# RoboticExplorationLab/TortoiseSat.jl

Hardware: AMD Instinct MI355X
Metric: AL-iLQR trajectory solves/sec (1000 knots) (higher is better)
Workload: dtype f64

## Files before the change

### tortoisesat.jl_amd/csrc/tsat_device.hpp

```cpp
#pragma once
#include <stdint.h>
#include "../../include/tortoise_hip.h"

#ifdef TSAT_EMU
#include <cmath>
namespace tsat_emu { int lane(); void sync(); void* lds(); double* xch(); }
#define TSAT_DEV inline
#define TSAT_PHASE inline
#define TSAT_FWD inline
#define TSAT_GLOBAL
#define TSAT_CONSTMEM
#define TSAT_LANE() (tsat_emu::lane())
#define TSAT_SYNC() (tsat_emu::sync())
#define TSAT_SYNC_LDS() (tsat_emu::sync())
#define TSAT_SCHED_FENCE() ((void)0)
#define TSAT_WAIT_LDS() ((void)0)
#define TSAT_NO_UNROLL
#define TSAT_ATOMIC_ADD(ptr, v) __atomic_fetch_add((ptr), (v), __ATOMIC_RELAXED)
#define TSAT_ATOMIC_LOAD(ptr) __atomic_load_n((ptr), __ATOMIC_RELAXED)
#define TSAT_UNIFORM_INT(x) (x)
#define TSAT_LANES_BELOW(n) (true)
#else
#define TSAT_DEV __device__ __forceinline__
#define TSAT_PHASE __device__ __noinline__
// ... 86 lines not shown
#elif defined(TSAT_JAC32)
  static constexpr int CHB = 64;
#elif defined(TSAT_DENSE)
  static constexpr int CHB = ES ? 29 : 25;
#else
  static constexpr int CHB = ES ? 64 : 55;
#endif
};
constexpr int KDW = 24, XUW = 10, LMW = 6, BSW = 9;
template <typename real> constexpr size_t pad16(size_t n) { return (n + (16 / sizeof(real)) - 1) / (16 / sizeof(real)) * (16 / sizeof(real)); }
template <typename real> constexpr size_t xu_stride(int NS) { return pad16<real>((size_t)NS * XUW); }
template <typename real> constexpr size_t kd_stride(int NS) { return (size_t)(NS - 1) * KDW; }
template <typename real> constexpr size_t lam_stride(int NS) { return pad16<real>((size_t)(NS - 1) * LMW); }
template <typename real> constexpr size_t u0_stride(int NS) { return (size_t)(NS - 1) * 3; }

template <typename real>
struct KArgs {
  int T, N, n_tab, max_ls;
  tsat_options opt;
  const real* P;
  const real* BT;
  const int* bidx;
  const int* nk;
  const real* U0;
  real* XU;
  real* KD;
  real* LAM;
  real* CAND;
  tsat_stats* stats;
  double* trace;
  int trace_rows;
  real* JW;
  int pk_few = 0;
  int ls_few = N_FEW, ls_hold = LS_HOLD;
  int suspend_at = 0;
  int* live = nullptr;
  int* susp_n = nullptr;
  int* susp_ids = nullptr;
  void* susp_state = nullptr;
};

constexpr int TSAT_JW_REALS_PER_4 = 16 * (4 * 84 + 4);

template <typename real>
struct TPtrs {
  TSAT_GLOBAL real* XU;
  TSAT_GLOBAL real* KD;
  TSAT_GLOBAL real* LAM;
  TSAT_GLOBAL real* CAND;
  const TSAT_GLOBAL real* bt;
  TSAT_GLOBAL real* XU0;
  int cur;
};
TSAT_DEV int cand_slab(int cur, int c) { return (c < cur) ? c : c + 1; }
template <typename real>
TSAT_DEV TSAT_GLOBAL real* slab_ptr(const TPtrs<real>& p, int N, int id) {
  return (id == 0) ? p.XU0 : p.CAND + (size_t)(id - 1) * (size_t)N * XUW;
}

constexpr int L_RED = 0;
constexpr int L_TR = L_RED + 64;
constexpr int TR_HJI = PSTRIDE, TR_HH = PSTRIDE + 9, TR_US = PSTRIDE + 10;
constexpr int L_NU = L_TR + 76;
constexpr int L_PC = L_NU + 8;
constexpr int L_ST = L_PC + 4;
constexpr int L_WT = L_ST + 72;
constexpr int L_HXX = L_WT + 90;
constexpr int L_HUX = L_HXX + 50;
constexpr int L_HUU = L_HUX + 24;
constexpr int L_KD = L_HUU + 10;
constexpr int L_ZERO = L_KD + 24;
constexpr int L_SINK = L_ZERO + 1;
constexpr int L_UNION = L_SINK + 1;
static_assert(L_UNION % 2 == 0, "phase buffers must stay 16-byte aligned");
constexpr int L_REC = L_UNION;
constexpr int GLDS = RPU * WAVE;
constexpr int BROW_UNITS = 4 / RPU;
constexpr int FB_KD = 0;
constexpr int FB_XU = FB_KD + ((CK * KDW + GLDS - 1) / GLDS) * GLDS;
constexpr int FB_BA = FB_XU + ((CK * XUW + GLDS - 1) / GLDS) * GLDS;
constexpr int FB_BB = FB_BA + ((CK * 3 * RPU + GLDS - 1) / GLDS) * GLDS;
constexpr int FB_SIZE = FB_BB + (BROW_UNITS == 2 ? ((CK * 3 * RPU + GLDS - 1) / GLDS) * GLDS : 0);
constexpr int CG = 2, KB = 4 * WAVE, KBS = KB + 2;
#if defined(TSAT_DENSE) || (defined(TSAT_F32) && TSAT_OCC >= 3)
constexpr int FWD_NBUF = 1;
#else
constexpr int FWD_NBUF = 2;
#endif
constexpr int L_FWD = L_UNION;
constexpr int L_FWD_END = L_FWD + (FWD_NBUF * FB_SIZE > CG * KBS ? FWD_NBUF * FB_SIZE : CG * KBS);
constexpr int L_BWD_RECV = (BwdCfg<0>::CHB * BwdCfg<0>::RECS > BwdCfg<1>::CHB * BwdCfg<1>::RECS
                               ? BwdCfg<0>::CHB * BwdCfg<0>::RECS : BwdCfg<1>::CHB * BwdCfg<1>::RECS);
constexpr int L_BWD_SOLVE = (L_BWD_RECV * (int)sizeof(jac_t) + (int)sizeof(cfg_real) - 1) / (int)sizeof(cfg_real);
#if !defined(TSAT_DENSE) && !defined(TSAT_F32)
constexpr int L_BWD_END = L_REC + (L_BWD_SOLVE > TV_CHB * TvRec::RECS ? L_BWD_SOLVE : TV_CHB * TvRec::RECS);
#else
constexpr int L_BWD_END = L_REC + L_BWD_SOLVE;
#endif
#if defined(TSAT_PACKED)
#ifndef TSAT_PK_LDS_BYTES
#define TSAT_PK_LDS_BYTES 20480
#endif
constexpr int LDS_REALS = (TSAT_PK_LDS_BYTES - ((sizeof(cfg_real) == 8) ? 0 : 64 * 8)) / (int)sizeof(cfg_real);
#else
constexpr int LDS_REALS = (L_FWD_END > L_BWD_END ? L_FWD_END : L_BWD_END);
#endif

constexpr int RED64_BYTES = (sizeof(cfg_real) == 8) ? 0 : 64 * 8;
constexpr int LDS_BYTES = LDS_REALS * (int)sizeof(cfg_real) + RED64_BYTES;
#ifndef TSAT_EMU
__shared__ __align__(16) unsigned char tsat_smem[LDS_BYTES];
#endif
template <typename real>
TSAT_DEV real* lds_base() {
  static_assert(sizeof(real) == sizeof(cfg_real), "the LDS carve-up is counted in the translation unit's storage type");
#ifdef TSAT_EMU
  return reinterpret_cast<real*>(tsat_emu::lds());
#else
  return reinterpret_cast<real*>(tsat_smem);
#endif
}
TSAT_DEV acc_t* red64() {
#ifdef TSAT_EMU
  unsigned char* b = reinterpret_cast<unsigned char*>(tsat_emu::lds());
#else
  unsigned char* b = tsat_smem;
#endif
  return reinterpret_cast<acc_t*>(b + (RED64_BYTES ? LDS_REALS * (int)sizeof(cfg_real) : L_RED * (int)sizeof(cfg_real)));
}

TSAT_DEV double* st64() {
#ifdef TSAT_EMU
  unsigned char* b = reinterpret_cast<unsigned char*>(tsat_emu::lds());
#else
  unsigned char* b = tsat_smem;
#endif
  return reinterpret_cast<double*>(b + L_ST * (int)sizeof(cfg_real));
}

template <typename real> TSAT_DEV real rsqrt_(real s);
#ifdef TSAT_EMU
template <> TSAT_DEV double rsqrt_<double>(double s) { return 1.0 / std::sqrt(s); }
template <> TSAT_DEV float rsqrt_<float>(float s) { return 1.0f / std::sqrt(s); }
TSAT_DEV double fabs_(double a) { return std::fabs(a); }
TSAT_DEV double fmax_(double a, double b) { return a > b ? a : b; }
TSAT_DEV double fmaxabs_(double a, double b) { const double c = std::fabs(b); return a > c ? a : c; }
TSAT_DEV double floor_(double a) { return std::floor(a); }
TSAT_DEV double fma_(double a, double b, double c) { return std::fma(a, b, c); }
TSAT_DEV double rcp_(double a) { return 1.0 / a; }
TSAT_DEV double sqrt_(double a) { return std::sqrt(a); }
TSAT_DEV double sin_(double a) { return std::sin(a); }
TSAT_DEV double cos_(double a) { return std::cos(a); }
TSAT_DEV double acos_(double a) { return std::acos(a); }
TSAT_DEV double asin_(double a) { return std::asin(a); }
TSAT_DEV double atan2_(double a, double b) { return std::atan2(a, b); }
TSAT_DEV double fmod_(double a, double b) { return std::fmod(a, b); }
TSAT_DEV double log_(double a) { return std::log(a); }
TSAT_DEV float fabs_(float a) { return std::fabs(a); }
TSAT_DEV float fmax_(float a, float b) { return a > b ? a : b; }
TSAT_DEV float fmaxabs_(float a, float b) { const float c = std::fabs(b); return a > c ? a : c; }
TSAT_DEV float rcp_(float a) { return 1.0f / a; }
TSAT_DEV float fma_(float a, float b, float c) { return std::fma(a, b, c); }
#else
template <> TSAT_DEV double rsqrt_<double>(double s) {
  const double y = __builtin_amdgcn_rsq(s);
  const double e = __builtin_fma(-(s * y), y, 1.0);
  const double p = __builtin_fma(0.375, e, 0.5) * e;
  return __builtin_fma(y, p, y);
}
template <> TSAT_DEV float rsqrt_<float>(float s) { return __builtin_amdgcn_rsqf(s); }
TSAT_DEV double fabs_(double a) { return __builtin_fabs(a); }
TSAT_DEV double fmax_(double a, double b) { double r; asm("v_max_f64 %0, %1, %2" : "=v"(r) : "v"(a), "v"(b)); return r; }
TSAT_DEV double fmaxabs_(double a, double b) { double r; asm("v_max_f64 %0, %1, |%2|" : "=v"(r) : "v"(a), "v"(b)); return r; }
TSAT_DEV double floor_(double a) { return __builtin_floor(a); }
TSAT_DEV double fma_(double a, double b, double c) { return __builtin_fma(a, b, c); }
TSAT_DEV double rcp_(double a) {
  const double y = __builtin_amdgcn_rcp(a);
  const double e = __builtin_fma(-a, y, 1.0);
  const double p = __builtin_fma(e, e, e);
  return __builtin_fma(y, p, y);
}
TSAT_DEV double sqrt_(double a) { return __builtin_sqrt(a); }
TSAT_DEV double sin_(double a) { return ::sin(a); }
TSAT_DEV double cos_(double a) { return ::cos(a); }
TSAT_DEV double acos_(double a) { return ::acos(a); }
TSAT_DEV double asin_(double a) { return ::asin(a); }
TSAT_DEV double atan2_(double a, double b) { return ::atan2(a, b); }
TSAT_DEV double fmod_(double a, double b) { return ::fmod(a, b); }
TSAT_DEV double log_(double a) { return ::log(a); }
TSAT_DEV float fabs_(float a) { return __builtin_fabsf(a); }
TSAT_DEV float fmax_(float a, float b) { float r; asm("v_max_f32 %0, %1, %2" : "=v"(r) : "v"(a), "v"(b)); return r; }
TSAT_DEV float fmaxabs_(float a, float b) { float r; asm("v_max_f32 %0, %1, |%2|" : "=v"(r) : "v"(a), "v"(b)); return r; }
TSAT_DEV float rcp_(float a) { return __builtin_amdgcn_rcpf(a); }
TSAT_DEV float fma_(float a, float b, float c) { return __builtin_fmaf(a, b, c); }
#endif
template <typename real> TSAT_DEV real dmm_(real a, real b, real c, real d) { return fma_(a, b, -(c * d)); }
template <typename real> TSAT_DEV real dot3_(real a0, real b0, real a1, real b1, real a2, real b2) { return fma_(a2, b2, fma_(a1, b1, a0 * b0)); }

#if defined(TSAT_PROFILE) && !defined(TSAT_EMU)
TSAT_DEV unsigned long long tick_() { return __builtin_amdgcn_s_memtime(); }
TSAT_DEV unsigned long long wall_() { return wall_clock64(); }
#else
TSAT_DEV unsigned long long tick_() { return 0ull; }
TSAT_DEV unsigned long long wall_() { return 0ull; }
#endif

template <typename real>
TSAT_DEV real sel7(const real a[7], int i) {
  real v = a[0];
  for (int m = 1; m < 7; ++m) v = (i == m) ? a[m] : v;
  return v;
}

template <typename real> TSAT_DEV real inf_() { return (real)__builtin_huge_val(); }

template <typename real>
TSAT_DEV void role_store(real* lds, int off, int sink, real v) {
#ifdef TSAT_EMU
  if (off == sink) return;
#else
  (void)sink;
#endif
  lds[off] = v;
}

template <typename real>
TSAT_DEV real wave_sum(real v, real* red) {
  const int lane = TSAT_LANE();
  for (int s = 1; s < WAVE; s <<= 1) {
    red[lane] = v;
    TSAT_SYNC_LDS();
    v = v + red[lane ^ s];
    TSAT_SYNC_LDS();
  }
  return v;
}
template <typename real>
TSAT_DEV real wave_max(real v, real* red) {
  const int lane = TSAT_LANE();
  for (int s = 1; s < WAVE; s <<= 1) {
    red[lane] = v;
    TSAT_SYNC_LDS();
    real o = red[lane ^ s];
    v = (o > v) ? o : v;
    TSAT_SYNC_LDS();
  }
  return v;
}
template <typename real>
TSAT_DEV real wave_bcast(real v, int src, real* red) {
  const int lane = TSAT_LANE();
  if (lane == src) red[0] = v;
  TSAT_SYNC_LDS();
  real r = red[0];
  TSAT_SYNC_LDS();
  return r;
}
template <typename real>
TSAT_DEV int wave_first(bool flag, real* red) {
  real v = flag ? (real)TSAT_LANE() : (real)WAVE;
  const int lane = TSAT_LANE();
  for (int s = 1; s < WAVE; s <<= 1) {
    red[lane] = v;
    TSAT_SYNC_LDS();
    real o = red[lane ^ s];
    v = (o < v) ? o : v;
    TSAT_SYNC_LDS();
  }
  return (int)v;
}

template <typename real>
struct Traj {
  real xf[7], Qd[7], Qfd[7], Rd[3], ulo[3], uhi[3];
  real J[9];
  real hJi[9];
  real h, hh, us;
  real usj;
  double tau0, dtau;
  int N, n_tab;
  const TSAT_GLOBAL real* bt;
};

template <typename real>
TSAT_DEV Traj<real> load_traj_at(const real* t, int N, int n_tab, const TSAT_GLOBAL real* bt) {
  Traj<real> tr;
  for (int i = 0; i < 7; ++i) { tr.xf[i] = t[P_XF + i]; tr.Qd[i] = t[P_QD + i]; tr.Qfd[i] = t[P_QFD + i]; }
  for (int i = 0; i < 3; ++i) { tr.Rd[i] = t[P_RD + i]; tr.ulo[i] = t[P_ULO + i]; tr.uhi[i] = t[P_UHI + i]; }
  for (int i = 0; i < 9; ++i) { tr.J[i] = t[P_J + i]; tr.hJi[i] = t[TR_HJI + i]; }
  tr.h = t[P_DT]; tr.hh = t[TR_HH]; tr.us = t[TR_US]; tr.usj = tr.us * tr.hJi[0];
  tr.tau0 = (double)t[P_TAU0] + (double)t[P_TAU0L]; tr.dtau = (double)t[P_DTAU] + (double)t[P_DTAUL];
  tr.N = N; tr.n_tab = n_tab; tr.bt = bt;
  return tr;
}
template <typename real>
TSAT_DEV Traj<real> load_traj(int N, int n_tab, const TSAT_GLOBAL real* bt) {
  return load_traj_at<real>(lds_base<real>() + L_TR, N, n_tab, bt);
// ... 440 lines not shown
  for (int i = 0; i < 7; ++i) x[i] = lds[L_TR + P_X0 + i];
  const TSAT_GLOBAL real* XUg = p.XU;
  const TSAT_GLOBAL real* KDg = p.KD;
  TSAT_GLOBAL real* Cg = slab_ptr<real>(p, N, cand_slab(p.cur, lane < n_cand ? lane : 0));
  int cur = 0;
  fwd_chunk_issue<real>(lds + L_FWD, KDg, XUg, tr, 0, (N - 1 < CK) ? N - 1 : CK, closed);
  TSAT_SYNC();
  for (int k0 = 0; k0 < N - 1; k0 += CK) {
    const int nk = (N - 1 - k0 < CK) ? (N - 1 - k0) : CK;
    const int kn = k0 + CK, nkn = (N - 1 - kn < CK) ? (N - 1 - kn) : CK;
    real* fb = lds + L_FWD + cur * FB_SIZE;
    real* fbn = lds + L_FWD + ((FWD_NBUF == 2) ? (1 - cur) : 0) * FB_SIZE;
    if (FWD_NBUF == 2 && nkn > 0) fwd_chunk_issue<real>(fbn, KDg, XUg, tr, kn, nkn, closed);
    auto knot = [&](const KnotIn<real>& kin, int kk) {
      const real* xu = kin.xu;
      real u[3] = {xu[7], xu[8], xu[9]};
      if (closed) {
        const real* kd = kin.kd;
        real dx[7];
        if (ES) {
          for (int i = 0; i < 3; ++i) dx[i] = x[i] - xu[i];
          const real s1 = xu[3], a1 = -xu[4], a2 = -xu[5], a3 = -xu[6];
          const real s2 = x[3], b1 = x[4], b2 = x[5], b3 = x[6];
          const real e0 = s1 * s2 - (a1 * b1 + a2 * b2 + a3 * b3);
          const real e1 = s1 * b1 + s2 * a1 + (a2 * b3 - a3 * b2);
          const real e2 = s1 * b2 + s2 * a2 + (a3 * b1 - a1 * b3);
          const real e3 = s1 * b3 + s2 * a3 + (a1 * b2 - a2 * b1);
          const real ir = rcp_((real)1 + e0);
          dx[3] = e1 * ir; dx[4] = e2 * ir; dx[5] = e3 * ir; dx[6] = 0;
        } else {
          for (int i = 0; i < 7; ++i) dx[i] = x[i] - xu[i];
        }
        for (int c = 0; c < 3; ++c) {
          real v = u[c];
          for (int j = 0; j < BwdCfg<ES>::NH; ++j) v += kd[c * 7 + j] * dx[j];
          u[c] = v + alpha * kd[21 + c];
        }
      }
      if (lane < n_cand) {
        TSAT_GLOBAL real* cr = Cg + (size_t)(k0 + kk) * XUW;
        for (int i = 0; i < 7; ++i) cr[i] = x[i];
        for (int c = 0; c < 3; ++c) cr[7 + c] = u[c];
      }
      real xn[7];
      rk_step<real, INTEG, DIAGJ, ES>(tr, x, u, kin.b0, kin.b1, kin.b2, xn);
      for (int i = 0; i < 7; ++i) x[i] = xn[i];
    };
#if defined(TSAT_DENSE) && !defined(TSAT_F32)
    for (int kk = 0; kk < nk; ++kk) {
      const KnotIn<real> A = fwd_knot_load<real>(fb, kk);
      knot(A, kk);
    }
#else
    KnotIn<real> A = fwd_knot_load<real>(fb, 0);
    for (int kk = 0; kk < nk; kk += 2) {
      TSAT_WAIT_LDS();
      const KnotIn<real> B = fwd_knot_load<real>(fb, (kk + 1 < nk) ? kk + 1 : kk);
      TSAT_SCHED_FENCE();
      knot(A, kk);
      if (kk + 1 < nk) {
        TSAT_WAIT_LDS();
        A = fwd_knot_load<real>(fb, (kk + 2 < nk) ? kk + 2 : kk + 1);
        TSAT_SCHED_FENCE();
        knot(B, kk + 1);
      }
    }
#endif
    if (nkn > 0) {
      if (FWD_NBUF == 1) {
        TSAT_SYNC_LDS();
        fwd_chunk_issue<real>(fbn, KDg, XUg, tr, kn, nkn, closed);
      }
      TSAT_SYNC();
      if (FWD_NBUF == 2) cur = 1 - cur;
    }
  }
  if (lane < n_cand) {
    TSAT_GLOBAL real* cr = Cg + (size_t)(N - 1) * XUW;
    for (int i = 0; i < 7; ++i) cr[i] = x[i];
    for (int c = 0; c < 3; ++c) cr[7 + c] = 0;
  }
}

template <typename real> struct CostIn { real lam[6], r[CG][XUW]; };
template <typename real>
TSAT_PHASE FwdOut<real> candidate_costs(TPtrs<real> p, int N, int c0, int nc, real mu, int term_mask, real max_state) {
  real* lds = lds_base<real>();
  const Traj<real> tr = load_traj<real>(N, 1, p.bt);
  const int lane = TSAT_LANE();
  HalfWeights<real> hw;
  for (int i = 0; i < 7; ++i) hw.hQd[i] = (real)0.5 * tr.Qd[i];
  for (int i = 0; i < 3; ++i) hw.hRd[i] = (real)0.5 * tr.Rd[i];
  hw.hmu = (real)0.5 * mu;
  real* L = lds + L_FWD;
  real am[CG];
  for (int c = 0; c < CG; ++c) am[c] = 0;
  acc_t J = 0;
  const int cme = (lane < nc) ? lane : 0;
  const TSAT_GLOBAL real* Cc[CG];
  for (int c = 0; c < CG; ++c) Cc[c] = slab_ptr<real>(p, N, cand_slab(p.cur, c0 + (c < nc ? c : 0)));
  const int S = (N + WAVE - 1) / WAVE;
  constexpr int SPB = KB / WAVE;
  auto load = [&](int st) {
    CostIn<real> in;
    const int k = st * WAVE + lane, kx = (k < N) ? k : N - 1, kl = (k < N - 1) ? k : 0;
    for (int e = 0; e < 6; ++e) in.lam[e] = p.LAM[(size_t)kl * LMW + e];
    for (int c = 0; c < CG; ++c)
      for (int e = 0; e < XUW; ++e) in.r[c][e] = (c < nc) ? Cc[c][(size_t)kx * XUW + e] : (real)0;
    return in;
  };
  auto step = [&](const CostIn<real>& in, int st) {
    const int k = st * WAVE + lane;
    real gate[6];
    for (int e = 0; e < 6; ++e) gate[e] = (in.lam[e] > 0) ? -inf_<real>() : (real)0;
    for (int c = 0; c < CG; ++c) {
      if (c >= nc) break;
      real a = am[c];
      if (k < N)
        for (int e = 0; e < 7; ++e) a = fmaxabs_(a, in.r[c][e]);
      if (k < N - 1) {
        for (int e = 7; e < 10; ++e) a = fmaxabs_(a, in.r[c][e]);
        L[c * KBS + (st % SPB) * WAVE + lane] = stage_cost_gated(tr, hw, in.r[c], in.r[c] + 7, in.lam, gate);
      }
      am[c] = a;
    }
    if ((st % SPB) == SPB - 1 || st == S - 1) {
      TSAT_SYNC_LDS();
      if (lane < nc) {
        const int k0 = (st / SPB) * KB;
        const int n = (N - 1 - k0 < KB) ? (N - 1 - k0) : KB;
        const real* Lc = L + cme * KBS;
        int kk = 0;
        for (; kk + 16 <= n; kk += 16) {
          real v[16];
          for (int e = 0; e < 16; ++e) v[e] = Lc[kk + e];
          for (int e = 0; e < 16; ++e) J += (acc_t)v[e];
        }
        for (; kk < n; ++kk) J += (acc_t)Lc[kk];
      }
      TSAT_SYNC_LDS();
    }
  };
  CostIn<real> A = load(0);
  for (int st = 0; st < S; st += 2) {
    const CostIn<real> B = load((st + 1 < S) ? st + 1 : st);
    step(A, st);
    if (st + 1 < S) {
      A = load((st + 2 < S) ? st + 2 : st + 1);
      step(B, st + 1);
    }
  }
  real amax = 0;
  for (int c = 0; c < CG; ++c) {
    if (c >= nc) break;
    const real m = wave_max(am[c], lds + L_RED);
    amax = (lane == c) ? m : amax;
  }
  real nu[7], xN[7];
  const TSAT_GLOBAL real* cN = slab_ptr<real>(p, N, cand_slab(p.cur, c0 + cme)) + (size_t)(N - 1) * XUW;
  for (int i = 0; i < 7; ++i) { nu[i] = lds[L_NU + i]; xN[i] = cN[i]; }
  J += (acc_t)term_cost(tr, xN, nu, mu, term_mask, true);
  FwdOut<real> out;
  out.J = J;
  out.ok = (lane < nc && (amax <= max_state) && (J == J)) ? 1 : 0;
  return out;
}


template <typename real>
TSAT_DEV void al_control_terms(const Traj<real>& tr, const real u[3], const real lam[6], real mu, real* lu_out, real* luu_out) {
  for (int c = 0; c < 3; ++c) {
    const real chi = u[c] - tr.uhi[c], clo = tr.ulo[c] - u[c];
    const real mhi = (chi > 0 || lam[c] > 0) ? mu : (real)0;
    const real mlo = (clo > 0 || lam[3 + c] > 0) ? mu : (real)0;
    real lu = fma_(tr.Rd[c], u[c], fma_(mhi, chi, lam[c]));
    lu = lu - fma_(mlo, clo, lam[3 + c]);
    lu_out[c] = lu;
    luu_out[c] = (tr.Rd[c] + mhi) + mlo;
  }
}

template <typename T, typename S>
TSAT_DEV Traj<T> traj_cast(const Traj<S>& a) {
  Traj<T> t;
  for (int i = 0; i < 7; ++i) { t.xf[i] = (T)a.xf[i]; t.Qd[i] = (T)a.Qd[i]; t.Qfd[i] = (T)a.Qfd[i]; }
  for (int i = 0; i < 3; ++i) { t.Rd[i] = (T)a.Rd[i]; t.ulo[i] = (T)a.ulo[i]; t.uhi[i] = (T)a.uhi[i]; }
  for (int i = 0; i < 9; ++i) { t.J[i] = (T)a.J[i]; t.hJi[i] = (T)a.hJi[i]; }
  t.h = (T)a.h; t.hh = (T)a.hh; t.us = (T)a.us; t.usj = (T)a.usj;
  t.tau0 = a.tau0; t.dtau = a.dtau; t.N = a.N; t.n_tab = a.n_tab; t.bt = nullptr;
  return t;
}
template <typename real, int INTEG, int DIAGJ, int ES, typename JP>
TSAT_DEV void knot_record(const Traj<real>& tr, const real x[7], const real u[3], const real lam[6], const real b0[3], const real b1[3],
                          const real b2[3], const real qn[4], real mu, JP rc) {
  using R = PkRec<ES>;
  if constexpr (sizeof(jac_t) == sizeof(real)) {
    if (!ES) rk_jacobian_cols<real, INTEG, DIAGJ, ES, JP, R::FSR>(tr, x, u, b0, b1, b2, rc, 0, 10);
    else rk_jacobian_es_cols<real, INTEG, DIAGJ, JP, R::FSR>(tr, x, u, b0, b1, b2, qn, rc, 0, 9);
  } else {
    const Traj<jac_t> tj = traj_cast<jac_t, real>(tr);
    jac_t xj[7], uj[3], c0[3], c1[3], c2[3], qj[4];
    for (int i = 0; i < 7; ++i) xj[i] = (jac_t)x[i];
    for (int i = 0; i < 3; ++i) { uj[i] = (jac_t)u[i]; c0[i] = (jac_t)b0[i]; c1[i] = (jac_t)b1[i]; c2[i] = (jac_t)b2[i]; }
    for (int i = 0; i < 4; ++i) qj[i] = (jac_t)qn[i];
    if (!ES) rk_jacobian_cols<jac_t, INTEG, DIAGJ, ES, JP, R::FSR>(tj, xj, uj, c0, c1, c2, rc, 0, 10);
    else rk_jacobian_es_cols<jac_t, INTEG, DIAGJ, JP, R::FSR>(tj, xj, uj, c0, c1, c2, qj, rc, 0, 9);
  }
  real lx[7];
  for (int i = 0; i < 7; ++i) lx[i] = tr.Qd[i] * (x[i] - tr.xf[i]);
  if (ES) {
    const real qk[4] = {x[3], x[4], x[5], x[6]};
    real o[3];
    gt_apply(qk, lx[3], lx[4], lx[5], lx[6], o);
    lx[3] = o[0]; lx[4] = o[1]; lx[5] = o[2];
    const real sq = qk[0], v0 = qk[1], v1 = qk[2], v2 = qk[3];
    const real G[4][3] = {{-v0, -v1, -v2}, {sq, -v2, v1}, {v2, sq, -v0}, {-v1, v0, sq}};
    int idx = 0;
    for (int j = 0; j < 3; ++j)
      for (int l = j; l < 3; ++l) {
        real acc = 0;
        for (int r = 0; r < 4; ++r) acc += G[r][j] * tr.Qd[3 + r] * G[r][l];
        rc[R::QQ + idx++] = (jac_t)acc;
      }
  }
  for (int i = 0; i < BwdCfg<ES>::NH; ++i) rc[R::LX + i] = (jac_t)lx[i];
  real lu[3], luu[3];
  al_control_terms(tr, u, lam, mu, lu, luu);
  for (int c = 0; c < 3; ++c) { rc[R::LU + c] = (jac_t)lu[c]; rc[R::LUU + c] = (jac_t)luu[c]; }
}

TSAT_DEV jac_t* rec_base() { return reinterpret_cast<jac_t*>(lds_base<cfg_real>() + L_REC); }

template <typename real, int INTEG, int DIAGJ, int ES>
TSAT_PHASE void jacobian_chunk(TPtrs<real> p, int N, int n_tab, int k0, int nk, real mu) {
  const int lane = TSAT_LANE();
  if (lane < nk) {
    const Traj<real> tr = load_traj<real>(N, n_tab, p.bt);
    const int k = k0 + lane;
    const TSAT_GLOBAL real* xu = p.XU + (size_t)k * XUW;
    real x[7], u[3], lam[6], b0[3], b1[3], b2[3], qn[4];
    for (int i = 0; i < 7; ++i) x[i] = xu[i];
    for (int c = 0; c < 3; ++c) u[c] = xu[7 + c];
    for (int c = 0; c < 6; ++c) lam[c] = p.LAM[(size_t)k * LMW + c];
    for (int i = 0; i < 4; ++i) qn[i] = xu[XUW + 3 + i];
    const TSAT_GLOBAL real* p0 = tr.bt + (size_t)brow_index(tr, k, 0.0) * 4;
    const TSAT_GLOBAL real* p1 = tr.bt + (size_t)brow_index(tr, k, 0.5) * 4;
    const TSAT_GLOBAL real* p2 = tr.bt + (size_t)brow_index(tr, k, 1.0) * 4;
    for (int c = 0; c < 3; ++c) { b0[c] = p0[c]; b1[c] = p1[c]; b2[c] = p2[c]; }
// ... 486 lines not shown
      g += m;
    }
  }
  g = wave_sum(g, lds + L_RED);
  return g / (real)(N - 1);
}

template <typename real>
TSAT_PHASE real todorov_gradient(const TSAT_GLOBAL real* XUs, const TSAT_GLOBAL real* KDg, int N) {
  real* lds = lds_base<real>();
  const int lane = TSAT_LANE();
  real g = 0;
  for (int k = lane; k < N - 1; k += WAVE) {
    real m = 0;
    for (int c = 0; c < 3; ++c) m = fmax_(m, fabs_(KDg[(size_t)k * KDW + 21 + c]) / (fabs_(XUs[(size_t)k * XUW + 7 + c]) + (real)1));
    g += m;
  }
  g = wave_sum(g, lds + L_RED);
  return g / (real)(N - 1);
}

template <typename real>
struct Resume {
  acc_t Jprev;
  real mu, rho, drho, grad, nu[7];
  int outer, it, djz, inner_iters, ls_trials, n_backward, n_forward, bp_restarts, fp_fails, trow;
  int cur;
  int since_deep;
};

template <typename real, int INTEG, int DIAGJ, int ES>
TSAT_DEV int solve_trajectory(const KArgs<real>& a, int traj, const Resume<real>* rs = nullptr) {
  real* lds = lds_base<real>();
  const int lane = TSAT_LANE();
  const tsat_options& o = a.opt;
  const int NS = a.N, n_tab = a.n_tab;
  const int N = a.nk ? a.nk[traj] : a.N;
  TPtrs<real> p;
  p.XU = (TSAT_GLOBAL real*)(a.XU + (size_t)traj * xu_stride<real>(NS));
  p.KD = (TSAT_GLOBAL real*)(a.KD + (size_t)traj * kd_stride<real>(NS));
  p.LAM = (TSAT_GLOBAL real*)(a.LAM + (size_t)traj * lam_stride<real>(NS));
  p.CAND = (TSAT_GLOBAL real*)(a.CAND + (size_t)traj * a.max_ls * xu_stride<real>(NS));
  p.bt = (const TSAT_GLOBAL real*)(a.BT + (size_t)a.bidx[traj] * n_tab * 4);
  p.XU0 = p.XU; p.cur = 0;
#define TSAT_ADOPT(slot) do { p.cur = cand_slab(p.cur, (slot)); p.XU = slab_ptr<real>(p, N, p.cur); } while (0)
  stage_traj<real>((const TSAT_GLOBAL real*)(a.P + (size_t)traj * PSTRIDE), (real)o.u_scale);

  const real* U0g = a.U0 + (size_t)traj * u0_stride<real>(NS);
  double* trace = a.trace ? a.trace + (size_t)traj * a.trace_rows * 8 : nullptr;
  int trow = 0;
  real mu = (real)o.penalty_init;
  const real max_state = (real)o.max_state;
  const int tmask = o.terminal_mask;
  int status = TSAT_MAX_OUTER, outer_iters = 0, inner_iters = 0, ls_trials = 0, n_backward = 0, n_forward = 0,
      bp_restarts = 0, fp_fails = 0;
  real grad = 0;
  int since_deep = LS_SHALLOW;
  const int ls_few = (a.ls_few >= 1) ? a.ls_few : N_FEW;
  unsigned long long pc_fwd = 0, pc_par = 0, pc_cost = 0;
  int n_cost = 0;
  bool start_ok = true;
  const unsigned long long t_s0 = tick_(), w_s0 = wall_();

  if (rs) {
    trow = rs->trow; mu = rs->mu; grad = rs->grad;
    p.cur = rs->cur; p.XU = slab_ptr<real>(p, N, p.cur);
    since_deep = rs->since_deep;
    inner_iters = rs->inner_iters; ls_trials = rs->ls_trials; n_backward = rs->n_backward; n_forward = rs->n_forward;
    bp_restarts = rs->bp_restarts; fp_fails = rs->fp_fails;
    if (lane < 7) lds[L_NU + lane] = rs->nu[lane];
    TSAT_SYNC();
  } else {
    for (int k = lane; k < N; k += WAVE) {
      for (int i = 0; i < 7; ++i) p.XU[(size_t)k * XUW + i] = 0;
      for (int c = 0; c < 3; ++c) p.XU[(size_t)k * XUW + 7 + c] = (k < N - 1) ? U0g[(size_t)k * 3 + c] : (real)0;
      if (k < N - 1)
        for (int c = 0; c < 6; ++c) p.LAM[(size_t)k * LMW + c] = 0;
    }
    TSAT_SYNC();
    forward_sweep<real, INTEG, DIAGJ, ES>(p, N, n_tab, 0, 1, 0);
    n_forward++;
    TSAT_SYNC();
    const FwdOut<real> f0 = candidate_costs<real>(p, N, 0, 1, mu, tmask, max_state);
    const acc_t J0 = wave_bcast(f0.J, 0, red64());
    const int ok0 = wave_first<real>(!f0.ok, lds + L_RED) > 0;
    TSAT_SYNC();
    TSAT_ADOPT(0);
    start_ok = ok0 && (J0 - J0 == 0);
  }
  if (!start_ok) {
    status = TSAT_DIVERGED;
  } else {
    bool resumed = rs != nullptr;
    for (int outer = rs ? rs->outer : 1; outer <= o.max_outer; ++outer) {
      acc_t Jprev;
      real rho = (real)o.reg_init, drho = 0;
      int djz = 0, it0 = 1;
      if (resumed) {
        Jprev = rs->Jprev; rho = rs->rho; drho = rs->drho; djz = rs->djz; it0 = rs->it;
        resumed = false;
      } else {
        Jprev = nominal_cost<real>(p, N, mu, tmask, 1);
      }
      bool regfail = false;
      for (int it = it0; it <= o.max_inner; ++it) {
#ifdef TSAT_PACKED
        if (rs && a.suspend_at && a.live) {
          int* seen = reinterpret_cast<int*>(lds + L_RED);
          TSAT_SYNC_LDS();
          if (lane == 0) seen[0] = TSAT_ATOMIC_LOAD(a.live);
          TSAT_SYNC_LDS();
          const int live_now = seen[0];
          TSAT_SYNC_LDS();
          if (live_now <= a.suspend_at) {
            if (lane == 0) {
              const int pos = TSAT_ATOMIC_ADD(a.susp_n, 1);
              a.susp_ids[pos] = traj;
              Resume<real>& r = reinterpret_cast<Resume<real>*>(a.susp_state)[pos];
              r.Jprev = Jprev; r.mu = mu; r.rho = rho; r.drho = drho; r.grad = grad;
              for (int i = 0; i < 7; ++i) r.nu[i] = lds[L_NU + i];
              r.outer = outer; r.it = it; r.djz = djz; r.inner_iters = inner_iters; r.ls_trials = ls_trials;
              r.n_backward = n_backward; r.n_forward = n_forward; r.bp_restarts = bp_restarts; r.fp_fails = fp_fails; r.trow = trow;
              r.cur = p.cur; r.since_deep = since_deep;
            }
            TSAT_SYNC();
            return 1;
          }
        }
#endif
        BwdOut<real> bw;
        for (;;) {
          n_backward++;
          bw = backward_sweep<real, INTEG, DIAGJ, ES>(p, N, n_tab, mu, rho, tmask);
          if (bw.pd_ok) break;
          bp_restarts++;
          drho = (drho * (real)o.reg_scale > (real)o.reg_scale) ? drho * (real)o.reg_scale : (real)o.reg_scale;
          rho = (rho * drho > (real)o.reg_min) ? rho * drho : (real)o.reg_min;
          if (rho > (real)o.reg_max) { regfail = true; break; }
        }
        if (regfail) break;
        const acc_t dV1 = bw.dV1, dV2 = bw.dV2;
        const real rho_used = rho;
        {
          const real inv = (real)1 / (real)o.reg_scale;
          drho = (drho / (real)o.reg_scale < inv) ? drho / (real)o.reg_scale : inv;
          const real r = rho * drho;
          rho = (r > (real)o.reg_min) ? r : (real)0;
        }
        TSAT_SYNC();
        const unsigned long long t_f0 = tick_();
        const int n_slots = (o.max_linesearch < a.max_ls) ? o.max_linesearch : a.max_ls;
        int jw = WAVE, slot = 0;
        acc_t Jw = 0;
        unsigned long long t_cost = 0;
        const bool keep_all = (a.ls_hold < 0) ? since_deep < LS_SHALLOW : since_deep <= a.ls_hold;
        int n_store = (keep_all || n_slots < ls_few) ? n_slots : ls_few;
        for (int shift = 0; shift < o.max_linesearch && jw == WAVE; shift += n_store, n_store = n_slots) {
          const int n_here = (o.max_linesearch - shift < n_store) ? o.max_linesearch - shift : n_store;
          forward_sweep<real, INTEG, DIAGJ, ES>(p, N, n_tab, 1, n_here, shift);
          n_forward++;
          TSAT_SYNC();
          const unsigned long long t_c0 = tick_();
          for (int c0 = 0; c0 < n_here && jw == WAVE; c0 += CG) {
            const int nc = (n_here - c0 < CG) ? n_here - c0 : CG;
            const FwdOut<real> fw = candidate_costs<real>(p, N, c0, nc, mu, tmask, max_state);
            n_cost++;
// ... 15 lines not shown
        }
        const unsigned long long t_f1 = tick_();
        pc_fwd += (t_f1 - t_f0) - t_cost;
        pc_par += t_cost;
        pc_cost += t_cost;
        acc_t J;
        TSAT_SYNC();
        if (jw >= ls_few - 1) since_deep = 0;
        else if (since_deep < LS_SHALLOW) since_deep++;
        if (jw < WAVE) {
          J = Jw;
          ls_trials += jw + 1;
          TSAT_ADOPT(slot);
          grad = todorov_gradient<real>(p.XU, p.KD, N);
        } else {
          J = Jprev;
          ls_trials += o.max_linesearch;
          fp_fails++;
          drho = (drho * (real)o.reg_scale > (real)o.reg_scale) ? drho * (real)o.reg_scale : (real)o.reg_scale;
          rho = (rho * drho > (real)o.reg_min) ? rho * drho : (real)o.reg_min;
          rho += (real)o.reg_fp;
          grad = todorov_gradient<real>(p.XU, p.KD, N);
        }
        TSAT_SYNC();
        pc_par += tick_() - t_f1;
        acc_t dJ = J - Jprev;
        dJ = dJ < 0 ? -dJ : dJ;
        if (trace && lane == 0 && trow < a.trace_rows) {
          double* r = trace + 8 * trow;
          r[0] = outer; r[1] = it; r[2] = (double)Jprev; r[3] = (double)J; r[4] = (jw < WAVE) ? jw : -1;
          r[5] = (double)rho_used; r[6] = (double)dV1; r[7] = (double)dV2;
#if defined(TSAT_PROFILE) && !defined(TSAT_EMU)
          r[7] = (double)wall_clock64();
#endif
        }
        trow++;
        Jprev = J;
        djz = (dJ == 0) ? djz + 1 : 0;
        inner_iters++;
        if (0 < dJ && dJ < (acc_t)o.cost_tol) break;
        if (grad < (real)o.grad_tol) break;
        if (djz > o.dj_counter_limit) break;
      }
      outer_iters = outer;
      const real cmax = violation_and_duals<real>(p, N, mu, tmask, 0, (real)o.dual_max);
      if (regfail) { status = TSAT_REG_FAIL; break; }
      if (cmax < (real)o.constraint_tol) { status = TSAT_CONVERGED; break; }
      if (outer == o.max_outer) break;
      (void)violation_and_duals<real>(p, N, mu, tmask, 1, (real)o.dual_max);
      if (lane < 7 && ((tmask >> lane) & 1)) {
        const real dmax = (real)o.dual_max;
        real v = lds[L_NU + lane] + mu * (p.XU[(size_t)(N - 1) * XUW + lane] - lds[L_TR + P_XF + lane]);
        v = v > -dmax ? v : -dmax; v = v < dmax ? v : dmax;
        lds[L_NU + lane] = v;
      }
      mu = (mu * (real)o.penalty_scale < (real)o.penalty_max) ? mu * (real)o.penalty_scale : (real)o.penalty_max;
      TSAT_SYNC();
    }
  }
  TSAT_SYNC();
  if (p.cur != 0) {
    for (int k = lane; k < N; k += WAVE)
      for (int i = 0; i < XUW; ++i) p.XU0[(size_t)k * XUW + i] = p.XU[(size_t)k * XUW + i];
    p.XU = p.XU0; p.cur = 0;
    TSAT_SYNC();
  }
  const real cmax = violation_and_duals<real>(p, N, mu, tmask, 0, (real)o.dual_max);
  const acc_t cost = nominal_cost<real>(p, N, mu, tmask, 0);
  const acc_t cost_al = nominal_cost<real>(p, N, mu, tmask, 1);
  if (lane == 0) {
    tsat_stats& st = a.stats[traj];
    st.status = status; st.outer_iters = outer_iters; st.inner_iters = inner_iters; st.ls_trials = ls_trials;
    st.n_backward = n_backward; st.n_forward = n_forward; st.bp_restarts = bp_restarts; st.fp_fails = fp_fails;
    st.cost = (double)cost; st.cost_al = (double)cost_al; st.c_max = (double)cmax; st.grad = (double)grad;
#ifdef TSAT_PROFILE
    if (trace && a.trace_rows > 0) {
      trace[0] = (double)pc_fwd; trace[1] = (double)lds[L_PC + 1]; trace[2] = (double)lds[L_PC + 2];
      trace[3] = (double)pc_par; trace[4] = (double)inner_iters; trace[5] = (double)n_backward;
#ifndef TSAT_PACKED
      trace[6] = (double)n_cost; trace[7] = (double)pc_cost;
      if (a.trace_rows > 1) {
        const unsigned long long w_s1 = wall_();
        trace[8] = (double)(tick_() - t_s0); trace[9] = (double)(w_s1 - w_s0); trace[10] = (double)w_s0; trace[11] = (double)w_s1;
      }
#endif
    }
#else
    (void)pc_fwd; (void)pc_par; (void)pc_cost; (void)n_cost; (void)t_s0; (void)w_s0;
#endif
  }
  return 0;
}

constexpr int P_QATT = 58;

template <typename real>
struct TvArgs {
  int T, N, n_tab, lin_sq, min_steps;
  real us, w_tol, ang_tol;
  const real* P;
  const real* BT;
  const int* bidx;
  const int* nk;
  const real* XUR;
  const real* NZ;
  int noise_mode;
  unsigned k0, k1;
  const long long* nid;
  int rate_as_written;
  real sg, sa, fa;
  real* KD;
  real* XS;
  tsat_tvlqr_stats* stats;
};

TSAT_DEV void philox4x32_10(unsigned k0, unsigned k1, unsigned c0, unsigned c1, unsigned c2, unsigned c3, unsigned out[4]) {
  for (int r = 0; r < 10; ++r) {
    const unsigned long long p0 = 0xD2511F53ull * c0, p1 = 0xCD9E8D57ull * c2;
    const unsigned n0 = (unsigned)(p1 >> 32) ^ c1 ^ k0, n1 = (unsigned)p1, n2 = (unsigned)(p0 >> 32) ^ c3 ^ k1, n3 = (unsigned)p0;
    c0 = n0; c1 = n1; c2 = n2; c3 = n3;
    k0 += 0x9E3779B9u; k1 += 0xBB67AE85u;
  }
  out[0] = c0; out[1] = c1; out[2] = c2; out[3] = c3;
}
template <typename real> TSAT_DEV real unit_open(unsigned w) { return ((real)w + (real)0.5) * (real)(1.0 / 4294967296.0); }
template <typename real> TSAT_DEV void box_muller(unsigned a, unsigned b, real& z0, real& z1) {
  const real r = sqrt_(-2 * log_(unit_open<real>(a))), th = (real)6.283185307179586476925 * unit_open<real>(b);
  z0 = r * cos_(th); z1 = r * sin_(th);
}
template <typename real>
TSAT_DEV void plant_noise(unsigned k0, unsigned k1, long long id, int knot, int stage, real sg, real sa, real fa, real nz[9]) {
  unsigned w0[4], w1[4], w2[4];
  const unsigned ilo = (unsigned)((unsigned long long)id & 0xFFFFFFFFull), ihi = (unsigned)((unsigned long long)id >> 32);
  philox4x32_10(k0, k1, ilo, ihi, (unsigned)knot, (unsigned)(4 * stage + 0), w0);
  philox4x32_10(k0, k1, ilo, ihi, (unsigned)knot, (unsigned)(4 * stage + 1), w1);
  philox4x32_10(k0, k1, ilo, ihi, (unsigned)knot, (unsigned)(4 * stage + 2), w2);
  real z[6];
  box_muller<real>(w0[0], w0[1], z[0], z[1]);
  box_muller<real>(w0[2], w0[3], z[2], z[3]);
  box_muller<real>(w1[0], w1[1], z[4], z[5]);
  for (int i = 0; i < 3; ++i) { nz[i] = sg * z[i]; nz[3 + i] = sa * z[3 + i]; }
  nz[6] = fa * unit_open<real>(w1[2]); nz[7] = fa * unit_open<real>(w1[3]); nz[8] = fa * unit_open<real>(w2[0]);
}

template <typename real, int DIAGJ>
TSAT_DEV void dyn_sim_h(const Traj<real>& tr, const real x[7], const real us[3], const real b[3],
                        bool noisy, const real nz[9], real k[7]) {
  real xx[7], bb[3];
  for (int i = 0; i < 7; ++i) xx[i] = x[i];
  for (int i = 0; i < 3; ++i) bb[i] = b[i];
  if (noisy) {
    const real rn = rsqrt_<real>(x[3] * x[3] + x[4] * x[4] + x[5] * x[5] + x[6] * x[6]);
    const real q0 = x[3] * rn, q1 = x[4] * rn, q2 = x[5] * rn, q3 = x[6] * rn;
    const real n0 = nz[3], n1 = nz[4], n2 = nz[5];
    const real th = sqrt_(n0 * n0 + n1 * n1 + n2 * n2);
    const real sh = sin_((real)0.5 * th) / th, ch = cos_((real)0.5 * th);
    const real d1 = n0 * sh, d2 = n1 * sh, d3 = n2 * sh;
    for (int i = 0; i < 3; ++i) { xx[i] = x[i] + nz[i]; bb[i] = b[i] + nz[6 + i]; }
    xx[3] = q0 * ch - (q1 * d1 + q2 * d2 + q3 * d3);
    xx[4] = q0 * d1 + ch * q1 + (q2 * d3 - q3 * d2);
    xx[5] = q0 * d2 + ch * q2 + (q3 * d1 - q1 * d3);
    xx[6] = q0 * d3 + ch * q3 + (q1 * d2 - q2 * d1);
  }
  StageBase<real> sb;
  dyn_h<real, DIAGJ>(tr, xx, us, bb, k, sb);
}
// ... 491 lines not shown
```

Baseline: 14580.

## Specialise candidate cost pass by candidate count and pipeline record loads

Splits candidate_costs into template instances for one or two candidates, so the per-candidate branches and zero-filled loads go away. Record loads become 2-wide vector loads issued one step ahead inside the step loop, and weights and bounds are made wave-uniform with readfirstlane so they can sit in scalar registers. The terminal state is stashed in LDS during the sweep rather than reread from global memory. Because the per-stage cost is now computed unconditionally, some padded lanes do extra work, and the LDS footprint grows slightly to hold the stashed terminal state. It also adds profiling counters for this phase.

After: 14890 (median of 6 runs). 2.2% higher.

```diff
diff --git a/tortoisesat.jl_amd/csrc/tsat_device.hpp b/tortoisesat.jl_amd/csrc/tsat_device.hpp
--- a/tortoisesat.jl_amd/csrc/tsat_device.hpp
+++ b/tortoisesat.jl_amd/csrc/tsat_device.hpp
@@ -192,13 +192,14 @@
 constexpr int FB_BB = FB_BA + ((CK * 3 * RPU + GLDS - 1) / GLDS) * GLDS;
 constexpr int FB_SIZE = FB_BB + (BROW_UNITS == 2 ? ((CK * 3 * RPU + GLDS - 1) / GLDS) * GLDS : 0);
 constexpr int CG = 2, KB = 4 * WAVE, KBS = KB + 2;
+constexpr int CC_XN = CG * KBS, CC_SIZE = CC_XN + CG * 8;
 #if defined(TSAT_DENSE) || (defined(TSAT_F32) && TSAT_OCC >= 3)
 constexpr int FWD_NBUF = 1;
 #else
 constexpr int FWD_NBUF = 2;
 #endif
 constexpr int L_FWD = L_UNION;
-constexpr int L_FWD_END = L_FWD + (FWD_NBUF * FB_SIZE > CG * KBS ? FWD_NBUF * FB_SIZE : CG * KBS);
+constexpr int L_FWD_END = L_FWD + (FWD_NBUF * FB_SIZE > CC_SIZE ? FWD_NBUF * FB_SIZE : CC_SIZE);
 constexpr int L_BWD_RECV = (BwdCfg<0>::CHB * BwdCfg<0>::RECS > BwdCfg<1>::CHB * BwdCfg<1>::RECS
                                ? BwdCfg<0>::CHB * BwdCfg<0>::RECS : BwdCfg<1>::CHB * BwdCfg<1>::RECS);
 constexpr int L_BWD_SOLVE = (L_BWD_RECV * (int)sizeof(jac_t) + (int)sizeof(cfg_real) - 1) / (int)sizeof(cfg_real);
@@ -215,6 +216,7 @@
 #else
 constexpr int LDS_REALS = (L_FWD_END > L_BWD_END ? L_FWD_END : L_BWD_END);
 #endif
+static_assert(L_FWD + CC_SIZE <= L_FWD_END && L_FWD + CC_SIZE <= LDS_REALS, "the cost blocks of candidate_costs fit this build's LDS block");
 
 constexpr int RED64_BYTES = (sizeof(cfg_real) == 8) ? 0 : 64 * 8;
 constexpr int LDS_BYTES = LDS_REALS * (int)sizeof(cfg_real) + RED64_BYTES;
@@ -323,6 +325,21 @@
 }
 
 template <typename real> TSAT_DEV real inf_() { return (real)__builtin_huge_val(); }
+
+template <typename real>
+TSAT_DEV real uniform_(real v) {
+#ifdef TSAT_EMU
+  return v;
+#else
+  if constexpr (sizeof(real) == 8) {
+    const unsigned long long u = __builtin_bit_cast(unsigned long long, v);
+    const unsigned lo = __builtin_amdgcn_readfirstlane((unsigned)u), hi = __builtin_amdgcn_readfirstlane((unsigned)(u >> 32));
+    return __builtin_bit_cast(real, ((unsigned long long)hi << 32) | lo);
+  } else {
+    return __builtin_bit_cast(real, (unsigned)__builtin_amdgcn_readfirstlane(__builtin_bit_cast(unsigned, v)));
+  }
+#endif
+}
 
 template <typename real>
 TSAT_DEV void role_store(real* lds, int off, int sink, real v) {
@@ -929,53 +946,68 @@
   }
 }
 
-template <typename real> struct CostIn { real lam[6], r[CG][XUW]; };
-template <typename real>
-TSAT_PHASE FwdOut<real> candidate_costs(TPtrs<real> p, int N, int c0, int nc, real mu, int term_mask, real max_state) {
+template <typename real>
+TSAT_DEV void load_record5(const TSAT_GLOBAL real* cr, real r[XUW]) {
+  static_assert(XUW == 2 * REC_STORES, "a record is REC_STORES pairs");
+#ifdef TSAT_EMU
+  for (int i = 0; i < XUW; ++i) r[i] = cr[i];
+#else
+  typedef real v2 __attribute__((ext_vector_type(2)));
+  typedef const TSAT_GLOBAL v2* gv2;
+  for (int i = 0; i < REC_STORES; ++i) {
+    const v2 v = ((gv2)cr)[i];
+    r[2 * i] = v.x; r[2 * i + 1] = v.y;
+  }
+#endif
+}
+template <typename real, int NC>
+TSAT_PHASE FwdOut<real> candidate_costs_n(TPtrs<real> p, int N_, int c0, real mu, int term_mask, real max_state) {
+  static_assert(1 <= NC && NC <= CG, "a pass takes up to CG candidates");
+  const int N = TSAT_UNIFORM_INT(N_);
   real* lds = lds_base<real>();
-  const Traj<real> tr = load_traj<real>(N, 1, p.bt);
+  Traj<real> tr = load_traj<real>(N, 1, p.bt);
   const int lane = TSAT_LANE();
   HalfWeights<real> hw;
-  for (int i = 0; i < 7; ++i) hw.hQd[i] = (real)0.5 * tr.Qd[i];
-  for (int i = 0; i < 3; ++i) hw.hRd[i] = (real)0.5 * tr.Rd[i];
-  hw.hmu = (real)0.5 * mu;
+  for (int i = 0; i < 7; ++i) { hw.hQd[i] = uniform_((real)0.5 * tr.Qd[i]); tr.xf[i] = uniform_(tr.xf[i]); }
+  for (int i = 0; i < 3; ++i) { hw.hRd[i] = uniform_((real)0.5 * tr.Rd[i]); tr.ulo[i] = uniform_(tr.ulo[i]); tr.uhi[i] = uniform_(tr.uhi[i]); }
+  hw.hmu = uniform_((real)0.5 * mu);
   real* L = lds + L_FWD;
-  real am[CG];
-  for (int c = 0; c < CG; ++c) am[c] = 0;
+  real am[NC];
+  for (int c = 0; c < NC; ++c) am[c] = 0;
   acc_t J = 0;
-  const int cme = (lane < nc) ? lane : 0;
-  const TSAT_GLOBAL real* Cc[CG];
-  for (int c = 0; c < CG; ++c) Cc[c] = slab_ptr<real>(p, N, cand_slab(p.cur, c0 + (c < nc ? c : 0)));
+  unsigned long long pc_sum = 0;
+  const int cme = (lane < NC) ? lane : 0;
+  const TSAT_GLOBAL real* Cc[NC];
+  for (int c = 0; c < NC; ++c) Cc[c] = slab_ptr<real>(p, N, cand_slab(p.cur, c0 + c));
   const int S = (N + WAVE - 1) / WAVE;
   constexpr int SPB = KB / WAVE;
-  auto load = [&](int st) {
-    CostIn<real> in;
-    const int k = st * WAVE + lane, kx = (k < N) ? k : N - 1, kl = (k < N - 1) ? k : 0;
-    for (int e = 0; e < 6; ++e) in.lam[e] = p.LAM[(size_t)kl * LMW + e];
-    for (int c = 0; c < CG; ++c)
-      for (int e = 0; e < XUW; ++e) in.r[c][e] = (c < nc) ? Cc[c][(size_t)kx * XUW + e] : (real)0;
-    return in;
+  auto load_lam = [&](real* lam, int st) {
+    const int k = st * WAVE + lane, kl = (k < N - 1) ? k : 0;
+    for (int e = 0; e < 6; ++e) lam[e] = p.LAM[(size_t)kl * LMW + e];
   };
-  auto step = [&](const CostIn<real>& in, int st) {
-    const int k = st * WAVE + lane;
+  auto load_rec = [&](real* r, int c, int st) {
+    const int k = st * WAVE + lane, kx = (k < N) ? k : N - 1;
+    load_record5<real>(Cc[c] + (size_t)kx * XUW, r);
+  };
+  auto step = [&](const real* lam, real (*r)[XUW], int st, int nx) {
+    const int b = st / SPB, q = st % SPB;
     real gate[6];
-    for (int e = 0; e < 6; ++e) gate[e] = (in.lam[e] > 0) ? -inf_<real>() : (real)0;
-    for (int c = 0; c < CG; ++c) {
-      if (c >= nc) break;
+    for (int e = 0; e < 6; ++e) gate[e] = (lam[e] > 0) ? -inf_<real>() : (real)0;
+    real* Lw = L + q * WAVE + lane;
+    for (int c = 0; c < NC; ++c) {
       real a = am[c];
-      if (k < N)
-        for (int e = 0; e < 7; ++e) a = fmaxabs_(a, in.r[c][e]);
-      if (k < N - 1) {
-        for (int e = 7; e < 10; ++e) a = fmaxabs_(a, in.r[c][e]);
-        L[c * KBS + (st % SPB) * WAVE + lane] = stage_cost_gated(tr, hw, in.r[c], in.r[c] + 7, in.lam, gate);
-      }
+      for (int e = 0; e < XUW; ++e) a = fmaxabs_(a, r[c][e]);
       am[c] = a;
-    }
-    if ((st % SPB) == SPB - 1 || st == S - 1) {
+      Lw[c * KBS] = stage_cost_gated(tr, hw, r[c], r[c] + 7, lam, gate);
+      if (st == S - 1 && st * WAVE + lane == N - 1)
+        for (int i = 0; i < 7; ++i) L[CC_XN + c * 8 + i] = r[c][i];
+      load_rec(r[c], c, nx);
+    }
+    if (q == SPB - 1 || st == S - 1) {
+      const unsigned long long t_a = tick_();
       TSAT_SYNC_LDS();
-      if (lane < nc) {
-        const int k0 = (st / SPB) * KB;
-        const int n = (N - 1 - k0 < KB) ? (N - 1 - k0) : KB;
+      if (lane < NC) {
+        const int n = (N - 1 - b * KB < KB) ? (N - 1 - b * KB) : KB;
         const real* Lc = L + cme * KBS;
         int kk = 0;
         for (; kk + 16 <= n; kk += 16) {
@@ -986,31 +1018,44 @@
         for (; kk < n; ++kk) J += (acc_t)Lc[kk];
       }
       TSAT_SYNC_LDS();
+      pc_sum += tick_() - t_a;
     }
   };
-  CostIn<real> A = load(0);
+  const unsigned long long t_l0 = tick_();
+  real lamA[6], lamB[6], r[NC][XUW];
+  load_lam(lamA, 0);
+  for (int c = 0; c < NC; ++c) load_rec(r[c], c, 0);
   for (int st = 0; st < S; st += 2) {
-    const CostIn<real> B = load((st + 1 < S) ? st + 1 : st);
-    step(A, st);
+    load_lam(lamB, (st + 1 < S) ? st + 1 : st);
+    step(lamA, r, st, (st + 1 < S) ? st + 1 : st);
     if (st + 1 < S) {
-      A = load((st + 2 < S) ? st + 2 : st + 1);
-      step(B, st + 1);
-    }
-  }
+      load_lam(lamA, (st + 2 < S) ? st + 2 : st + 1);
+      step(lamB, r, st + 1, (st + 2 < S) ? st + 2 : st + 1);
+    }
+  }
+#if defined(TSAT_PROFILE) && !defined(TSAT_EMU)
+  if (lane == 0) { lds[L_PC + 0] += (real)((tick_() - t_l0) - pc_sum); lds[L_PC + 3] += (real)pc_sum; }
+#else
+  (void)t_l0; (void)pc_sum;
+#endif
   real amax = 0;
-  for (int c = 0; c < CG; ++c) {
-    if (c >= nc) break;
+  for (int c = 0; c < NC; ++c) {
     const real m = wave_max(am[c], lds + L_RED);
     amax = (lane == c) ? m : amax;
   }
   real nu[7], xN[7];
-  const TSAT_GLOBAL real* cN = slab_ptr<real>(p, N, cand_slab(p.cur, c0 + cme)) + (size_t)(N - 1) * XUW;
-  for (int i = 0; i < 7; ++i) { nu[i] = lds[L_NU + i]; xN[i] = cN[i]; }
+  for (int i = 0; i < 7; ++i) { nu[i] = lds[L_NU + i]; xN[i] = L[CC_XN + cme * 8 + i]; }
   J += (acc_t)term_cost(tr, xN, nu, mu, term_mask, true);
   FwdOut<real> out;
   out.J = J;
-  out.ok = (lane < nc && (amax <= max_state) && (J == J)) ? 1 : 0;
+  out.ok = (lane < NC && (amax <= max_state) && (J == J)) ? 1 : 0;
   return out;
+}
+template <typename real>
+TSAT_DEV FwdOut<real> candidate_costs(TPtrs<real> p, int N, int c0, int nc, real mu, int term_mask, real max_state) {
+  static_assert(CG == 2, "one instance per group width");
+  if (TSAT_UNIFORM_INT(nc) >= 2) return candidate_costs_n<real, 2>(p, N, c0, mu, term_mask, max_state);
+  return candidate_costs_n<real, 1>(p, N, c0, mu, term_mask, max_state);
 }
 
 
@@ -1663,6 +1708,9 @@
     n_forward++;
     TSAT_SYNC();
     const FwdOut<real> f0 = candidate_costs<real>(p, N, 0, 1, mu, tmask, max_state);
+#if defined(TSAT_PROFILE) && !defined(TSAT_EMU)
+    if (lane == 0) lds[L_PC + 0] = lds[L_PC + 3] = 0;
+#endif
     const acc_t J0 = wave_bcast(f0.J, 0, red64());
     const int ok0 = wave_first<real>(!f0.ok, lds + L_RED) > 0;
     TSAT_SYNC();
@@ -1844,6 +1892,7 @@
       if (a.trace_rows > 1) {
         const unsigned long long w_s1 = wall_();
         trace[8] = (double)(tick_() - t_s0); trace[9] = (double)(w_s1 - w_s0); trace[10] = (double)w_s0; trace[11] = (double)w_s1;
+        trace[12] = (double)lds[L_PC + 0]; trace[13] = (double)lds[L_PC + 3];
       }
 #endif
     }
```
